# Thealexbarney/VGAudio

Hardware: AMD Instinct MI355X
Metric: Msamples/s encoded (GC-ADPCM, 4096 ch) at 1/2/4/8 GPUs; % HBM roofline (higher is better)
Workload: dtype int32; 1 GPU; BASELINE configs[1]: 4096 mono channels x 48 kHz x 60 s GC-ADPCM coefficient search + encode per GPU; parallelism=units sharded x1, channels_per_gpu=4096, samples_per_channel=2880000, bit_exact_channels_checked=0

## Files before the change

### vgaudio_amd/csrc/gc_encode_core.hpp

```cpp
#pragma once
#include <cstdint>

#if defined(__HIPCC__)
#define VGA_HD __host__ __device__ __forceinline__
#else
#define VGA_HD inline
#endif

#if defined(__HIP_DEVICE_COMPILE__)
#define VGA_MUL24(a, b) __mul24((a), (b))
#define VGA_OPAQUE(v) asm("" : "+v"(v))
#define VGA_OPAQUE_S(v) asm("" : "+s"(v))
static __device__ __forceinline__ uint32_t vga_square24(int e)
{
    uint32_t r;
    asm("v_mul_i32_i24 %0, %1, %1" : "=v"(r) : "v"(e));
    return r;
}
#else
#define VGA_MUL24(a, b) ((a) * (b))
#define VGA_OPAQUE(v) ((void)0)
#define VGA_OPAQUE_S(v) ((void)0)
#endif

// ... 173 lines not shown
    const float f = (float)d;
    if (f >= 2147483648.0f) return 2147483647;
    return (int)f;
#endif
}

VGA_HD uint32_t pack16(int lo, int hi) { return ((uint32_t)lo & 0xFFFFu) | ((uint32_t)hi << 16); }
VGA_HD int pair_lo(uint32_t v) { return (int)(int16_t)(v & 0xFFFFu); }
VGA_HD int pair_hi(uint32_t v) { return (int)v >> 16; }
VGA_HD int dot2_i16(uint32_t a, uint32_t b, int acc)
{
#if defined(__HIP_DEVICE_COMPILE__)
    typedef short s16x2 __attribute__((ext_vector_type(2)));
    return __builtin_amdgcn_sdot2(__builtin_bit_cast(s16x2, a), __builtin_bit_cast(s16x2, b), acc, true);
#else
    const int64_t v = (int64_t)pair_lo(a) * pair_lo(b) + (int64_t)pair_hi(a) * pair_hi(b) + (int64_t)acc;
    return v > 2147483647ll ? 2147483647 : (v < -2147483648ll ? (int)-2147483648ll : (int)v);
#endif
}
VGA_HD uint32_t sat_pack16(int lo, int hi)
{
#if defined(__HIP_DEVICE_COMPILE__)
    return __builtin_bit_cast(uint32_t, __builtin_amdgcn_cvt_pk_i16(lo, hi));
#else
    return pack16(clamp16i(lo), clamp16i(hi));
#endif
}
VGA_HD uint32_t pk_sub_sat_i16(uint32_t a, uint32_t b)
{
#if defined(__HIP_DEVICE_COMPILE__)
    typedef short s16x2 __attribute__((ext_vector_type(2)));
    return __builtin_bit_cast(uint32_t, __builtin_elementwise_sub_sat(__builtin_bit_cast(s16x2, a), __builtin_bit_cast(s16x2, b)));
#else
    return pack16(clamp16i(pair_lo(a) - pair_lo(b)), clamp16i(pair_hi(a) - pair_hi(b)));
#endif
}
VGA_HD int dot2_i16_wrap(uint32_t a, uint32_t b)
{
#if defined(__HIP_DEVICE_COMPILE__)
    typedef short s16x2 __attribute__((ext_vector_type(2)));
    return __builtin_amdgcn_sdot2(__builtin_bit_cast(s16x2, a), __builtin_bit_cast(s16x2, b), 0, false);
#else
    return (int)((uint32_t)(pair_lo(a) * pair_lo(b)) + (uint32_t)(pair_hi(a) * pair_hi(b)));
#endif
}
VGA_HD int numer_adjust(int N, int D_is_pos)
{
    VGA_OPAQUE(D_is_pos);
    return (int)((uint32_t)N + (uint32_t)VGA_MUL24(D_is_pos, 2047));
}
VGA_HD int head_distance_numer(int in2048p, int P)
{
    const int N = (int)((uint32_t)in2048p - (uint32_t)P);
    return numer_adjust(N, (int)((uint32_t)(1024 - P) >> 31)) >> 11;
}
VGA_HD void pack_row(const int (&x)[16], uint32_t (&xw)[7])
{
#if defined(__HIP_DEVICE_COMPILE__)
#pragma unroll
#endif
    for (int i = 0; i < 7; i++) xw[i] = pack16(x[2 + 2 * i], x[3 + 2 * i]);
}
VGA_HD void unpack_row(const uint32_t (&xw)[7], uint32_t hist, int (&x)[16])
{
    x[0] = pair_lo(hist);
    x[1] = pair_hi(hist);
#if defined(__HIP_DEVICE_COMPILE__)
#pragma unroll
#endif
    for (int i = 0; i < 7; i++) { x[2 + 2 * i] = pair_lo(xw[i]); x[3 + 2 * i] = pair_hi(xw[i]); }
}

VGA_HD int predicted_p1024(uint32_t h, uint32_t cpair)
{
    int k1024 = 1024;
    VGA_OPAQUE_S(k1024);
    return dot2_i16(h, cpair, k1024);
}
template <bool WIDE_TOTAL, bool NO_ROUND = false, bool HAVE_P0 = false>
VGA_HD PassOut pass_fast_core_t(const uint32_t (&xw)[7], uint32_t hist, const int (&in2048p)[14], int c0, int c1, int scale_power,
                                int P0 = 0)
{
    PassOut r;
    uint64_t total64 = 0;
    const int k = scale_power + 11;
    const int km11 = scale_power;
    int bias = (1 << (k - 1)) - 1;
    VGA_OPAQUE(bias);
    const uint32_t cpair = pack16(c1, c0);
    int k1024 = 1024;
    VGA_OPAQUE_S(k1024);
    int total = 0;
    int umax = 0, umin = 0;
    int u_prev = 0;
    uint32_t h = hist;
    int w_prev = pair_hi(hist);
#if defined(__HIP_DEVICE_COMPILE__)
#pragma unroll
#endif
    for (int s = 0; s < 14; s++) {
        const int P = (HAVE_P0 && s == 0) ? P0 : dot2_i16(h, cpair, k1024);
        const int d = (int)((uint32_t)in2048p[s] - (uint32_t)P);
        const int rd = NO_ROUND ? d : round_through_f32(d);
        const int u = (int)((uint32_t)rd + (uint32_t)bias + ((uint32_t)d >> 31)) >> k;
        const int q = imin(imax(u, -8), 7);
        if (s & 1) {
            umax = imax(imax(umax, u_prev), u);
            umin = imin(imin(umin, u_prev), u);
        }
        u_prev = u;
        r.q[s] = q;
        const int w = (P >> 11) + (int)((uint32_t)q << km11);
        h = sat_pack16(w_prev, w);
        w_prev = w;
        if (WIDE_TOTAL) {
            const int e = ((s & 1) ? pair_hi(xw[s >> 1]) : pair_lo(xw[s >> 1])) - pair_hi(h);
#if defined(__HIP_DEVICE_COMPILE__)
            total64 += (uint64_t)vga_square24(e);
#else
            total64 += (uint64_t)((int64_t)e * (int64_t)e);
#endif
        } else if (s & 1) {
            const uint32_t epk = pk_sub_sat_i16(xw[s >> 1], h);
            total = dot2_i16(epk, epk, total);
        }
    }
    r.hist_pair = h;
    const int ov = imax(imax(umax - 7, -8 - umin), 0);
    const int ac0 = c0 < 0 ? -c0 : c0, ac1 = c1 < 0 ? -c1 : c1;
    r.exact = ac0 + ac1 <= 32767 && (WIDE_TOTAL || (ov <= 12383 && (((2 * ov + 1) << (k - 11)) <= 24766)));
    r.total = WIDE_TOTAL ? total64 : (uint64_t)(uint32_t)total;
    r.max_overflow = ov;
    r.o12 = pair_lo(h); r.o13 = pair_hi(h);
    return r;
}
VGA_HD PassOut pass_fast_core(const uint32_t (&xw)[7], uint32_t hist, const int (&in2048p)[14], int c0, int c1, int scale_power)
{
    return pass_fast_core_t<false>(xw, hist, in2048p, c0, c1, scale_power);
}
VGA_HD PassOut pass_fast_core_no_round(const uint32_t (&xw)[7], uint32_t hist, const int (&in2048p)[14], int c0, int c1,
                                       int scale_power)
{
    return pass_fast_core_t<false, true>(xw, hist, in2048p, c0, c1, scale_power);
}
VGA_HD bool pass_no_round_is_exact(int scale_power, int max_overflow)
{
    return scale_power <= 9 && max_overflow < (1 << (13 - scale_power)) - 8;
}
VGA_HD PassOut pass_fast_core_wide(const uint32_t (&xw)[7], uint32_t hist, const int (&in2048p)[14], int c0, int c1,
                                   int scale_power)
{
    return pass_fast_core_t<true>(xw, hist, in2048p, c0, c1, scale_power);
}
constexpr uint64_t PACKED_SUM_CAP = 1ull << 28;
VGA_HD bool needs_exact_sum(uint64_t total, bool known_exact) { return !known_exact && total >= PACKED_SUM_CAP; }
VGA_HD PassOut pass_fast_core(const int (&x)[16], uint32_t hist, const int (&in2048p)[14], int c0, int c1, int scale_power)
{
    uint32_t xw[7];
    pack_row(x, xw);
    return pass_fast_core_t<false>(xw, hist, in2048p, c0, c1, scale_power);
}
VGA_HD PassOut pass_fast_core_no_round(const int (&x)[16], uint32_t hist, const int (&in2048p)[14], int c0, int c1,
                                       int scale_power)
{
    uint32_t xw[7];
    pack_row(x, xw);
    return pass_fast_core_t<false, true>(xw, hist, in2048p, c0, c1, scale_power);
}
VGA_HD PassOut pass_fast_core_wide(const int (&x)[16], uint32_t hist, const int (&in2048p)[14], int c0, int c1,
                                   int scale_power)
{
    uint32_t xw[7];
    pack_row(x, xw);
    return pass_fast_core_t<true>(xw, hist, in2048p, c0, c1, scale_power);
}
template <bool NO_ROUND>
VGA_HD PassOut pass_fast_core_exact_sum(const int (&x)[16], const int (&in2048p)[14], int c0, int c1, int scale_power)
{
    uint32_t xw[7];
    pack_row(x, xw);
    const uint32_t hist = pack16(x[0], x[1]);
    PassOut r = pass_fast_core_t<false, NO_ROUND>(xw, hist, in2048p, c0, c1, scale_power);
    const int ac0 = c0 < 0 ? -c0 : c0, ac1 = c1 < 0 ? -c1 : c1;
    if (ac0 + ac1 <= 32767 && needs_exact_sum(r.total, r.exact))
        r.total = pass_fast_core_t<true>(xw, hist, in2048p, c0, c1, scale_power).total;
    return r;
}
VGA_HD PassOut pass_fast_core(const int (&x)[16], const int (&)[14], const int (&in2048p)[14], int c0, int c1, int scale_power)
{
    return pass_fast_core_exact_sum<false>(x, in2048p, c0, c1, scale_power);
}
VGA_HD PassOut pass_fast_core_no_round(const int (&x)[16], const int (&)[14], const int (&in2048p)[14], int c0, int c1,
                                       int scale_power)
{
    return pass_fast_core_exact_sum<true>(x, in2048p, c0, c1, scale_power);
}
VGA_HD PassOut pass_fast_core_wide(const int (&x)[16], const int (&)[14], const int (&in2048p)[14], int c0, int c1,
                                   int scale_power)
{
    return pass_fast_core_wide(x, pack16(x[0], x[1]), in2048p, c0, c1, scale_power);
}

VGA_HD PassOut pass_fast(const int (&x)[16], int c0, int c1, int scale_power)
{
    int in2048p[14];
#if defined(__HIP_DEVICE_COMPILE__)
#pragma unroll
#endif
    for (int s = 0; s < 14; s++) in2048p[s] = x[s + 2] * 2048 + 1024;
    return pass_fast_core(x, pack16(x[0], x[1]), in2048p, c0, c1, scale_power);
}

struct Resolve {
    bool final_a;
    bool final_b;
    int resume_sp;
};

VGA_HD Resolve resolve_candidates(int s1, int ov_a, int ov_b)
{
    Resolve z;
    z.final_a = z.final_b = false;
    z.resume_sp = 0;
    const int sp_a = apply_bumps(s1, ov_a);
    if (!(sp_a < 12 && ov_a > 1)) { z.final_a = true; return z; }
    if (sp_a != s1) { z.resume_sp = sp_a; return z; }
    const int s2 = s1 + 1;
    const int sp_b = apply_bumps(s2, ov_b);
    if (!(sp_b < 12 && ov_b > 1)) { z.final_b = true; return z; }
    z.resume_sp = sp_b;
    return z;
}

VGA_HD Resolve resolve_candidates_nobump(int s1, int ov_a, int ov_b)
{
    Resolve z;
    z.final_a = !(s1 < 12 && ov_a > 1);
    z.final_b = !z.final_a && !(s1 + 1 < 12 && ov_b > 1);
    z.resume_sp = s1 + 1;
    return z;
}

VGA_HD PassOut resume_passes_core(const int (&x)[16], const int (&in2048p)[14], int c0, int c1, int scale_power,
                                  int &final_sp)
{
    PassOut r;
    bool at_max;
    do {
        scale_power++;
        at_max = scale_power >= 12;
        r = pass_fast_core(x, pack16(x[0], x[1]), in2048p, c0, c1, scale_power);
        if (!r.exact) r = pass_literal(x, c0, c1, scale_power);
        scale_power = apply_bumps(scale_power, r.max_overflow);
    } while (scale_power < 12 && r.max_overflow > 1 && !at_max);
    final_sp = scale_power;
    return r;
}

VGA_HD PassOut resume_passes(const int (&x)[16], int c0, int c1, int scale_power, int &final_sp)
{
    PassOut r;
    bool at_max;
    do {
        scale_power++;
        at_max = scale_power >= 12;
        r = pass_fast(x, c0, c1, scale_power);
        if (!r.exact) r = pass_literal(x, c0, c1, scale_power);
        scale_power = apply_bumps(scale_power, r.max_overflow);
    } while (scale_power < 12 && r.max_overflow > 1 && !at_max);
    final_sp = scale_power;
    return r;
}

}
}
```

### vgaudio_amd/csrc/gc_encode_kernel.hip

```cpp
#include "common.hpp"
#include "gc_encode_core.hpp"
#include "gcadpcm_kernels.hpp"
#include "seams.hpp"

#include <cstdio>
#include <cstdlib>

namespace vga {
namespace gc {

constexpr int DPP_QUAD_XOR1 = 0xB1;
constexpr int DPP_QUAD_XOR2 = 0x4E;
constexpr int DPP_ROW_HALF_MIRROR = 0x141;
constexpr int DPP_ROW_MIRROR = 0x140;

template <int CTRL>
__device__ __forceinline__ int dpp(int v)
{
    return __builtin_amdgcn_update_dpp(0, v, CTRL, 0xF, 0xF, true);
}

__device__ __forceinline__ unsigned umin32(unsigned a, unsigned b) { return a < b ? a : b; }

template <class Op>
__device__ __forceinline__ unsigned row16_reduce(unsigned v, Op op)
{
    v = op(v, (unsigned)dpp<DPP_QUAD_XOR1>((int)v));
    v = op(v, (unsigned)dpp<DPP_QUAD_XOR2>((int)v));
    v = op(v, (unsigned)dpp<DPP_ROW_HALF_MIRROR>((int)v));
    v = op(v, (unsigned)dpp<DPP_ROW_MIRROR>((int)v));
    return v;
}


#ifdef VGA_DEBUG_TIMESTAMPS
__device__ unsigned long long g_vga_enc_ts[1 << 16];
extern "C" int vga_debug_encode_timestamps(unsigned long long *out, int n)
{
    return (int)hipMemcpyFromSymbol(out, HIP_SYMBOL(g_vga_enc_ts), (size_t)n * sizeof(unsigned long long));
}
#endif
__device__ unsigned long long g_vga_gc_stats[8];
extern "C" int vga_testing_gc_encode_stats(unsigned long long *out8, int reset)
{
    if (hipDeviceSynchronize() != hipSuccess) return -1;
    if (out8 && hipMemcpyFromSymbol(out8, HIP_SYMBOL(g_vga_gc_stats), 8 * sizeof(unsigned long long)) != hipSuccess) return -1;
#ifdef VGA_GC_STATS
    if (out8) out8[7] = 1;
#else
    if (out8) out8[7] = 0;
#endif
    if (reset) {
        const unsigned long long zero[8] = {0, 0, 0, 0, 0, 0, 0, 0};
        if (hipMemcpyToSymbol(HIP_SYMBOL(g_vga_gc_stats), zero, sizeof zero) != hipSuccess) return -1;
    }
    return 0;
}
constexpr int SW = 2;
constexpr int ENC_THREADS = 64 * (SW + 1);
#ifndef VGA_GC_ENCODER_PRIO
#define VGA_GC_ENCODER_PRIO 3
#endif
#ifndef VGA_GC_HELPER_PRIO
#define VGA_GC_HELPER_PRIO 0
#endif
template <int CPW>
struct Lay {
    static constexpr int CS = CPW * SW;
    static constexpr int TF = 64 / CS;
};
template <int CS, int TF>
struct GcTileT {
    uint32_t xw[CS][TF][8];
    int in2048p[CS][TF][16];
    uint32_t pre[CS][TF][8];
};
typedef short short2v __attribute__((ext_vector_type(2)));
struct XW7 { uint32_t v[7]; };

#define VGA_COLD __device__ __forceinline__

VGA_COLD int prescan_sequential_cold(XW7 xs, uint32_t hist, int c0, int c1)
{
    int x[16];
    unpack_row(xs.v, hist, x);
    return prescan_sequential(x, c0, c1);
}

#ifdef VGA_GC_R05_COLD
#define VGA_COLD_OPAQUE(v) ((void)0)
#else
#define VGA_COLD_OPAQUE(v) VGA_OPAQUE(v)
#endif
struct ColdState {
    uint32_t xw[7];
    int mp[14];
    uint32_t hist;
    int c0, c1, s1;
    int generic, start, drop, wide, resume;
    int bump_a, ov_a, ov_b;
};
struct ColdOut { PassOut r; int final_sp; int fin; int sum_exact; };
__device__ __forceinline__
ColdOut encode_frame_cold(ColdState st, PassOut r, int final_sp, int fin)
{
    uint32_t xw[7];
    int mp[14];
#pragma unroll
    for (int i = 0; i < 7; i++) xw[i] = st.xw[i];
#pragma unroll
    for (int i = 0; i < 14; i++) mp[i] = st.mp[i];
    int sum_exact = 0;
    if (st.drop) fin = 0;
    if (__any(st.generic != 0)) {
        if (st.generic) {
            int xg[16];
            unpack_row(xw, st.hist, xg);
#pragma unroll
            for (int i = 0; i < 16; i++) VGA_COLD_OPAQUE(xg[i]);
            const int start = st.start != -100 ? st.start
                                               : (st.bump_a ? apply_bumps(st.s1, st.ov_a) : apply_bumps(st.s1 + 1, st.ov_b));
            r = resume_passes(xg, st.c0, st.c1, start, final_sp);
            fin = 1;
            sum_exact = 1;
        }
    }
    if (st.wide) fin = 1;
    if (__any(st.resume != 0)) {
        if (st.resume) {
            int sp = st.s1 + 1;
            for (;;) {
                sp++;
#if defined(VGA_GC_NO_FAST_PASSES) || defined(VGA_GC_NO_FAST_THIRD)
                bool short_pass = false;
#else
                bool short_pass = !__any(sp > 9);
#endif
                if (short_pass) {
                    r = pass_fast_core_no_round(xw, st.hist, mp, st.c0, st.c1, sp);
                    short_pass = !__any(!pass_no_round_is_exact(sp, r.max_overflow));
                }
                if (!short_pass) r = pass_fast_core(xw, st.hist, mp, st.c0, st.c1, sp);
                const bool cap = sp >= 12;
                if ((unsigned)r.max_overflow > (cap ? 3u : 248u)) {
                    int xg[16];
                    unpack_row(xw, st.hist, xg);
#pragma unroll
                    for (int i = 0; i < 16; i++) VGA_COLD_OPAQUE(xg[i]);
                    r = resume_passes(xg, st.c0, st.c1, sp - 1, final_sp);
                    sum_exact = 1;
                    break;
                }
                final_sp = sp;
                if (cap || r.max_overflow <= 1) break;
            }
            fin = 1;
        }
    }
    ColdOut o;
    o.r = r;
    o.final_sp = final_sp;
    o.fin = fin;
    o.sum_exact = sum_exact;
    return o;
}

template <bool REPAIR, int CPW, bool RAGGED>
__device__ __forceinline__ void gc_encode_piece(
    const int bx, const int by,
    const int16_t *__restrict__ pcm, int64_t pcm_pitch, int nch, int total_samples, const Pieces seg,
    const int16_t *__restrict__ coefs, const int16_t *__restrict__ hist1,
    const int16_t *__restrict__ hist2, uint8_t *__restrict__ adpcm, int64_t adpcm_pitch, int16_t *__restrict__ seg_state,
    const int *__restrict__ first_open, const Ragged &rg)
{
    constexpr bool repair = REPAIR;
    constexpr int CS = Lay<CPW>::CS, TF = Lay<CPW>::TF;
    using GcTile = GcTileT<CS, TF>;
    int64_t first_frame = seg.first(by);
    int repair_piece = 0;
    if (repair) {
        int k = SEAM_OPEN_LIMIT;
        for (int g = 0; g < CS; g++) {
            const int slot = bx * CS + g;
            if (slot < nch) {
                const int c = RAGGED ? rg.order[slot] : slot;
                k = first_open[c] < k ? first_open[c] : k;
            }
        }
        if (!is_open(k)) return;
        repair_piece = k;
        first_frame = seg.first(k);
    }
    const int total_wg = RAGGED ? rg.length[rg.order[bx * CS]] : total_samples;
    if (first_frame * 14 >= total_wg) return;
    const int64_t piece_samples = repair ? (int64_t)0x7fffffff : (int64_t)seg.frames(by) * 14;
    auto piece_samples_of = [&](int total) {
        const int64_t rem = (int64_t)total - first_frame * 14;
        return (int)(rem < 0 ? 0 : (rem < piece_samples ? rem : piece_samples));
    };
    pcm += first_frame * 14;
    adpcm += first_frame * 8;
    __shared__ GcTile s_tile[2];
    __shared__ int4 s_out[2][CS][TF][4];
    __shared__ int s_ncold[SW];
    const int tid = threadIdx.x;
    const int wave = tid >> 6;
    const bool helper = wave == SW;
    const int lane = tid & 63;
    constexpr int LPC = 64 / CPW;
    int grp = helper ? lane / TF : wave * CPW + lane / LPC;
    const int l16 = lane & (LPC - 1);
    const int hfr = lane % TF;
    const int slot_raw = bx * CS + grp;
    const bool live = slot_raw < nch;
    const int slot = live ? slot_raw : nch - 1;
    const int ch = RAGGED ? rg.order[slot] : slot;
    const int16_t *src = pcm + (RAGGED ? rg.pcm_off[ch] : (int64_t)ch * pcm_pitch);
    uint8_t *dst = adpcm + (RAGGED ? rg.adpcm_off[ch] : (int64_t)ch * adpcm_pitch);

    const int sample_count = piece_samples_of(RAGGED ? rg.length[ch] : total_samples);
    const int full_frames = sample_count / 14;
    const int tail = sample_count - full_frames * 14;
    const int frames = full_frames + (tail ? 1 : 0);
    const int frames_wg = RAGGED ? (piece_samples_of(total_wg) + 13) / 14 : frames;
    const int tiles = (frames_wg + TF - 1) / TF;

    if (helper) {
        __builtin_amdgcn_s_setprio(VGA_GC_HELPER_PRIO);
        uint32_t cpk[8];
#pragma unroll
        for (int p = 0; p < 8; p++)
            cpk[p] = (uint32_t)(uint16_t)coefs[ch * 16 + 2 * p + 1] | ((uint32_t)(uint16_t)coefs[ch * 16 + 2 * p] << 16);
        auto prepare = [&](int tile) {
            const int fr = RAGGED ? imax(imin(tile * TF + hfr, frames - 1), 0) : imin(tile * TF + hfr, frames - 1);
            int in[14];
            uint32_t w[7];
            if (fr < full_frames) {
                const uint32_t *p32 = reinterpret_cast<const uint32_t *>(src + (int64_t)fr * 14);
#pragma unroll
                for (int i = 0; i < 7; i++) w[i] = p32[i];
#pragma unroll
                for (int i = 0; i < 7; i++) {
                    in[2 * i] = (int)(int16_t)(w[i] & 0xFFFF);
                    in[2 * i + 1] = (int)w[i] >> 16;
                }
            } else {
#pragma unroll
                for (int s = 0; s < 14; s++) in[s] = (s < tail) ? (int)src[(int64_t)fr * 14 + s] : 0;
#pragma unroll
                for (int i = 0; i < 7; i++) w[i] = (uint32_t)(in[2 * i] & 0xFFFF) | ((uint32_t)in[2 * i + 1] << 16);
            }
            GcTile &T = s_tile[tile & 1];
            uint4 *xr = reinterpret_cast<uint4 *>(&T.xw[grp][hfr][0]);
            xr[0] = make_uint4(w[0], w[1], w[2], w[3]);
            xr[1] = make_uint4(w[4], w[5], w[6], 0u);
            int4 *qr = reinterpret_cast<int4 *>(&T.in2048p[grp][hfr][0]);
            qr[0] = make_int4(in[0] * 2048 + 1024, in[1] * 2048 + 1024, in[2] * 2048 + 1024, in[3] * 2048 + 1024);
            qr[1] = make_int4(in[4] * 2048 + 1024, in[5] * 2048 + 1024, in[6] * 2048 + 1024, in[7] * 2048 + 1024);
            qr[2] = make_int4(in[8] * 2048 + 1024, in[9] * 2048 + 1024, in[10] * 2048 + 1024, in[11] * 2048 + 1024);
            qr[3] = make_int4(in[12] * 2048 + 1024, in[13] * 2048 + 1024, 0, 0);
            uint32_t pair[12];
#pragma unroll
            for (int k = 0; k < 12; k++)
                pair[k] = (k & 1) ? __builtin_amdgcn_alignbit(w[(k + 1) / 2], w[(k - 1) / 2], 16) : w[k / 2];
            uint32_t pre[8];
#pragma unroll
            for (int p = 0; p < 8; p++) {
                int dmax = 0, dmin = 0;
#ifdef VGA_GC_ABLATE_HELPER_PRESCAN
                dmax = in[2 + p] & 1023;
                dmin = -(in[3 + p] & 1023);
#else
#pragma unroll
                for (int k = 0; k < 12; k++) {
                    const int predicted = div2048(__builtin_amdgcn_sdot2(__builtin_bit_cast(short2v, pair[k]),
                                                                         __builtin_bit_cast(short2v, cpk[p]), 0, false));
                    const int d = in[k + 2] - predicted;
                    dmax = imax(dmax, d);
                    dmin = imin(dmin, d);
                }
#endif
                pre[p] = (uint32_t)(clamp16i(dmax) & 0xFFFF) | ((uint32_t)clamp16i(dmin) << 16);
            }
            uint4 *pr = reinterpret_cast<uint4 *>(&T.pre[grp][hfr][0]);
            pr[0] = make_uint4(pre[0], pre[1], pre[2], pre[3]);
            pr[1] = make_uint4(pre[4], pre[5], pre[6], pre[7]);
        };
        auto flush = [&](int tile) {
            const int fr = tile * TF + hfr;
            if (!live || fr >= frames) return;
            const int4 *rec = &s_out[tile & 1][grp][hfr][0];
            const int4 r0 = rec[0], r1 = rec[1], r2 = rec[2], r3 = rec[3];
            const int q[14] = {r0.x, r0.y, r0.z, r0.w, r1.x, r1.y, r1.z, r1.w, r2.x, r2.y, r2.z, r2.w, r3.x, r3.y};
            uint2 v;
            pack_frame(q, r3.z, r3.w, v.x, v.y);
            if (fr < full_frames) {
                *reinterpret_cast<uint2 *>(dst + (int64_t)fr * 8) = v;
            } else {
                const int nbytes = (tail + 2 + 1) / 2;
                const uint64_t both = ((uint64_t)v.y << 32) | v.x;
                for (int b = 0; b < nbytes; b++) dst[(int64_t)fr * 8 + b] = (uint8_t)(both >> (8 * b));
            }
        };
        if (tiles > 0) prepare(0);
        __syncthreads();
        for (int tile = 0; tile < tiles; tile++) {
            if (tile + 1 < tiles) prepare(tile + 1);
            if (tile > 0) flush(tile - 1);
            __syncthreads();
        }
        if (tiles > 0) flush(tiles - 1);
        return;
    }

    __builtin_amdgcn_s_setprio(VGA_GC_ENCODER_PRIO);
    int p = CPW == 4 ? l16 >> 1 : l16;
    const bool cand_b = CPW == 4 && (l16 & 1) != 0;
    const int c0 = coefs[ch * 16 + 2 * p];
    const int c1 = coefs[ch * 16 + 2 * p + 1];
    const bool coef_ok = (c0 < 0 ? -c0 : c0) + (c1 < 0 ? -c1 : c1) <= 32767;
    int h0 = hist2 ? hist2[ch] : 0;
    int h1 = hist1 ? hist1[ch] : 0;
    if (repair) {
        h0 = seg_state[((int64_t)(repair_piece - 1) * nch + ch) * 2];
        h1 = seg_state[((int64_t)(repair_piece - 1) * nch + ch) * 2 + 1];
    } else if (by > 0 && (!RAGGED || frames > 0)) {
        h0 = src[-2];
        h1 = src[-1];
    }
    uint32_t hpk = pack16(h0, h1);

    if (lane == 0) s_ncold[wave] = 0;
    struct Row { uint32_t xw[7]; int mp[14]; uint32_t pre; };
    auto read_row = [&](const GcTile &T, int j, Row &R) {
        const uint4 *xr = reinterpret_cast<const uint4 *>(&T.xw[grp][j][0]);
        const uint4 a0 = xr[0], a1 = xr[1];
        asm volatile("" ::"v"(a1.w));
        uint32_t *xw = R.xw;
        xw[0] = a0.x; xw[1] = a0.y; xw[2] = a0.z; xw[3] = a0.w; xw[4] = a1.x; xw[5] = a1.y; xw[6] = a1.z;
        const int4 *qr = reinterpret_cast<const int4 *>(&T.in2048p[grp][j][0]);
        const int4 e0 = qr[0], e1 = qr[1], e2 = qr[2], e3 = qr[3];
        asm volatile("" ::"v"(e3.z), "v"(e3.w));
        int *mp = R.mp;
        mp[0] = e0.x; mp[1] = e0.y; mp[2] = e0.z; mp[3] = e0.w; mp[4] = e1.x; mp[5] = e1.y; mp[6] = e1.z; mp[7] = e1.w;
        mp[8] = e2.x; mp[9] = e2.y; mp[10] = e2.z; mp[11] = e2.w; mp[12] = e3.x; mp[13] = e3.y;
        R.pre = T.pre[grp][j][p];
    };
    auto pack = [](const uint32_t (&xw)[7]) {
        XW7 xs;
#pragma unroll
        for (int i = 0; i < 7; i++) xs.v[i] = xw[i];
        return xs;
    };
    const uint32_t cpk = pack16(c1, c0);
    const bool head_numer = __builtin_amdgcn_ballot_w64(!coef_ok) == 0;
    auto prescan_head = [&](const Row &R, int &d0, int &d1, int &P0) __attribute__((always_inline)) {
        P0 = predicted_p1024(hpk, cpk);
        if (__builtin_expect(head_numer, 1)) {
            d0 = head_distance_numer(R.mp[0], P0);
            d1 = head_distance_numer(R.mp[1], predicted_p1024(__builtin_amdgcn_alignbit(R.xw[0], hpk, 16), cpk));
        } else {
            d0 = pair_lo(R.xw[0]) - div2048(dot2_i16_wrap(hpk, cpk));
            d1 = pair_hi(R.xw[0]) - div2048(dot2_i16_wrap(__builtin_amdgcn_alignbit(R.xw[0], hpk, 16), cpk));
        }
    };
    auto first_scale = [&](const Row &R, int d0, int d1) __attribute__((always_inline)) -> int {
        const int dmax = imax(imax((int)(int16_t)(R.pre & 0xFFFF), d0), d1);
        const int dmin = imin(imin((int)R.pre >> 16, d0), d1);
        int sum, pos;
        int s1 = first_scale_power_nt(dmax, dmin, sum, pos);
        if (__builtin_expect(__builtin_amdgcn_ballot_w64(sum == 0) != 0, 0)) {
            if (sum == 0 && first_scale_tie(pos)) s1 = first_scale_power_from_md(prescan_sequential_cold(pack(R.xw), hpk, c0, c1));
        }
        return s1;
    };

    auto encode_frame = [&](Row &R, int buf, int j, bool upd) {
        const uint32_t (&xw)[7] = R.xw;
        int s1, P0;
        {
            int d0, d1;
            prescan_head(R, d0, d1, P0);
            s1 = first_scale(R, d0, d1);
        }
        int final_sp = imin(s1 + (cand_b ? 1 : 0), 12);
        const bool at_cap = final_sp >= 12;
        const unsigned ov_limit = at_cap ? 3u : 248u;
        PassOut r = pass_fast_core_t<false, false, true>(xw, hpk, R.mp, c0, c1, final_sp, P0);
        const bool rare = !coef_ok || (!at_cap && (unsigned)r.max_overflow > ov_limit);
        const int eff = at_cap ? 0 : r.max_overflow;
        const int eff_other = dpp<DPP_QUAD_XOR1>(eff);
        bool fin = eff < 2 && (eff_other | (cand_b ? 0 : 2)) >= 2;
        const bool resume = !cand_b && imin(eff, eff_other) >= 2;
        const bool inexact = fin && at_cap && (unsigned)r.max_overflow > ov_limit;
        constexpr unsigned SAT = (1u << 28) - 1;
        auto argmin32 = [&](const PassOut &r, bool fin, bool &sat) __attribute__((always_inline)) -> int {
            const unsigned tot = umin32((unsigned)(r.total >> 32) ? SAT : (unsigned)r.total, SAT);
            const unsigned key = fin ? ((tot << 4) | (unsigned)l16) : 0xFFFFFFFFu;
            const unsigned best = row16_reduce(key, [](unsigned a, unsigned b) { return a < b ? a : b; });
            sat = __any((best >> 4) >= SAT);
            return (int)(best & 15u);
        };
        auto argmin64 = [&](uint64_t total, bool fin) __attribute__((always_inline)) -> int {
            uint64_t key = fin ? ((total << 4) | (uint64_t)l16) : ~0ull;
#define VGA_MIN64_STAGE(CTRL)                                                          \
            {                                                                          \
                const unsigned olo = (unsigned)dpp<CTRL>((int)(uint32_t)key);          \
                const unsigned ohi = (unsigned)dpp<CTRL>((int)(uint32_t)(key >> 32));  \
                const uint64_t okey = ((uint64_t)ohi << 32) | olo;                     \
                key = okey < key ? okey : key;                                         \
            }
            VGA_MIN64_STAGE(DPP_QUAD_XOR1)
            VGA_MIN64_STAGE(DPP_QUAD_XOR2)
            VGA_MIN64_STAGE(DPP_ROW_HALF_MIRROR)
            VGA_MIN64_STAGE(DPP_ROW_MIRROR)
#undef VGA_MIN64_STAGE
            return (int)(key & 15u);
        };
        auto commit = [&](const PassOut &r, int final_sp, int winner) __attribute__((always_inline)) {
            const bool won = l16 == winner;
            const unsigned pay = row16_reduce(won ? r.hist_pair : 0u,
                                              [](unsigned a, unsigned b) { return a | b; });
            if (won) {
                int4 *rec = &s_out[buf][grp][j][0];
                rec[0] = make_int4(r.q[0], r.q[1], r.q[2], r.q[3]);
                rec[1] = make_int4(r.q[4], r.q[5], r.q[6], r.q[7]);
                rec[2] = make_int4(r.q[8], r.q[9], r.q[10], r.q[11]);
                rec[3] = make_int4(r.q[12], r.q[13], p, final_sp);
            }
            if (!RAGGED || upd) hpk = pay;
        };
        bool sat = false;
        const int winner32 = argmin32(r, fin && !inexact, sat);
        if (__builtin_expect(__any(rare || resume || inexact) || sat, 0)) {
#ifdef VGA_GC_STATS
            if (lane == 0) atomicAdd(&s_ncold[wave], 1);
#endif
            ColdState st;
#pragma unroll
            for (int i = 0; i < 7; i++) st.xw[i] = xw[i];
#pragma unroll
            for (int i = 0; i < 14; i++) st.mp[i] = R.mp[i];
            st.hist = hpk;
            st.c0 = c0; st.c1 = c1; st.s1 = s1;
            const bool redo = __any(rare);
            st.generic = redo && !cand_b; st.start = s1 - 1; st.drop = redo && cand_b;
            st.wide = !redo && inexact; st.resume = !redo && resume;
            st.bump_a = 0; st.ov_a = 0; st.ov_b = 0;
            const ColdOut o = encode_frame_cold(st, r, final_sp, fin);
            bool sat2 = false;
            int winner = argmin32(o.r, o.fin != 0, sat2);
            if (sat2) {
                uint64_t total = o.r.total;
                if (o.fin != 0 && needs_exact_sum(total, o.sum_exact != 0))
                    total = pass_fast_core_wide(xw, hpk, R.mp, c0, c1, o.final_sp).total;
                winner = argmin64(total, o.fin != 0);
            }
            commit(o.r, o.final_sp, winner);
        } else
            commit(r, final_sp, winner32);
    };

    auto encode_frame8 = [&](Row &R, int buf, int j, bool upd) {
        const uint32_t (&xw)[7] = R.xw;
        int s1, P0;
        {
            int d0, d1;
            prescan_head(R, d0, d1, P0);
            s1 = first_scale(R, d0, d1);
        }
        const int sp_a = imin(s1, 12), sp_b = imin(s1 + 1, 12);
        PassOut ra, rb;
#ifdef VGA_GC_NO_FAST_PASSES
        bool short_passes = false;
#else
        bool short_passes = !__any(sp_b > 9);
#endif
        if (short_passes) {
            rb = pass_fast_core_t<false, true, true>(xw, hpk, R.mp, c0, c1, sp_b, P0);
            ra = pass_fast_core_t<false, true, true>(xw, hpk, R.mp, c0, c1, sp_a, P0);
            const bool trusted = !coef_ok || (pass_no_round_is_exact(sp_a, ra.max_overflow) && pass_no_round_is_exact(sp_b, rb.max_overflow));
            short_passes = !__any(!trusted);
        }
        if (!short_passes) {
            rb = pass_fast_core_t<false, false, true>(xw, hpk, R.mp, c0, c1, sp_b, P0);
            ra = pass_fast_core_t<false, false, true>(xw, hpk, R.mp, c0, c1, sp_a, P0);
        }
        const bool cap_a = sp_a >= 12, cap_b = sp_b >= 12;
        const int eff_a = cap_a ? 0 : ra.max_overflow, eff_b = cap_b ? 0 : rb.max_overflow;
        const bool fin_a = eff_a < 2;
        const bool bump_a = !cap_a && (unsigned)ra.max_overflow > 248u;
        const bool bump_b = !fin_a && !cap_b && (unsigned)rb.max_overflow > 248u;
        const bool generic = !coef_ok || bump_a || bump_b;
        const bool inexact = !generic && (fin_a ? (cap_a && (unsigned)ra.max_overflow > 3u) : (cap_b && (unsigned)rb.max_overflow > 3u));
#ifdef VGA_GC_ABLATE_THIRD_TRIPS
        const bool resume = false;
#else
        const bool resume = !generic && !fin_a && eff_b >= 2;
#endif
        PassOut r;
#pragma unroll
        for (int i = 0; i < 14; i++) r.q[i] = fin_a ? ra.q[i] : rb.q[i];
        r.total = fin_a ? ra.total : rb.total;
        r.hist_pair = fin_a ? ra.hist_pair : rb.hist_pair;
        r.max_overflow = fin_a ? ra.max_overflow : rb.max_overflow;
        r.o12 = r.o13 = 0;
        r.exact = true;
        const int final_sp = fin_a ? sp_a : sp_b;
        constexpr unsigned SAT = (1u << 28) - 1;
        auto argmin32 = [&](const PassOut &r, bool fin, bool &sat) __attribute__((always_inline)) -> int {
            const unsigned tot = umin32((unsigned)(r.total >> 32) ? SAT : (unsigned)r.total, SAT);
            unsigned key = fin ? ((tot << 3) | (unsigned)p) : 0xFFFFFFFFu;
            key = umin32(key, (unsigned)dpp<DPP_QUAD_XOR1>((int)key));
            key = umin32(key, (unsigned)dpp<DPP_QUAD_XOR2>((int)key));
            key = umin32(key, (unsigned)dpp<DPP_ROW_HALF_MIRROR>((int)key));
            sat = __any((key >> 3) >= SAT);
            return (int)(key & 7u);
        };
        auto argmin64 = [&](uint64_t total, bool fin) __attribute__((always_inline)) -> int {
            uint64_t key = fin ? ((total << 3) | (uint64_t)p) : ~0ull;
#define VGA_MIN64_STAGE(CTRL)                                                          \
            {                                                                          \
                const unsigned olo = (unsigned)dpp<CTRL>((int)(uint32_t)key);          \
                const unsigned ohi = (unsigned)dpp<CTRL>((int)(uint32_t)(key >> 32));  \
                const uint64_t okey = ((uint64_t)ohi << 32) | olo;                     \
                key = okey < key ? okey : key;                                         \
            }
            VGA_MIN64_STAGE(DPP_QUAD_XOR1)
            VGA_MIN64_STAGE(DPP_QUAD_XOR2)
            VGA_MIN64_STAGE(DPP_ROW_HALF_MIRROR)
#undef VGA_MIN64_STAGE
            return (int)(key & 7u);
        };
        auto commit = [&](const PassOut &r, int final_sp, int winner) __attribute__((always_inline)) {
            const bool won = p == winner;
            unsigned pay = won ? r.hist_pair : 0u;
            pay |= (unsigned)dpp<DPP_QUAD_XOR1>((int)pay);
            pay |= (unsigned)dpp<DPP_QUAD_XOR2>((int)pay);
            pay |= (unsigned)dpp<DPP_ROW_HALF_MIRROR>((int)pay);
            if (won) {
                int4 *rec = &s_out[buf][grp][j][0];
                rec[0] = make_int4(r.q[0], r.q[1], r.q[2], r.q[3]);
                rec[1] = make_int4(r.q[4], r.q[5], r.q[6], r.q[7]);
                rec[2] = make_int4(r.q[8], r.q[9], r.q[10], r.q[11]);
                rec[3] = make_int4(r.q[12], r.q[13], p, final_sp);
            }
            if (!RAGGED || upd) hpk = pay;
        };
        bool sat = false;
        const int winner32 = argmin32(r, !(generic || resume || inexact), sat);
        if (__builtin_expect(__any(generic || resume || inexact) || sat, 0)) {
#ifdef VGA_GC_STATS
            if (lane == 0) atomicAdd(&s_ncold[wave], 1);
#endif
            ColdState st;
#pragma unroll
            for (int i = 0; i < 7; i++) st.xw[i] = xw[i];
#pragma unroll
            for (int i = 0; i < 14; i++) st.mp[i] = R.mp[i];
            st.hist = hpk;
            st.c0 = c0; st.c1 = c1; st.s1 = s1;
            st.generic = generic; st.drop = 0; st.wide = inexact; st.resume = resume;
#ifdef VGA_GC_R05_COLD
            st.start = !coef_ok ? s1 - 1 : (bump_a ? apply_bumps(s1, ra.max_overflow) : apply_bumps(s1 + 1, rb.max_overflow));
#else
            st.start = !coef_ok ? s1 - 1 : -100;
#endif
            st.bump_a = bump_a; st.ov_a = ra.max_overflow; st.ov_b = rb.max_overflow;
            const ColdOut o = encode_frame_cold(st, r, final_sp, (generic || resume) ? 0 : 1);
            bool sat2 = false;
            int winner = argmin32(o.r, o.fin != 0, sat2);
            if (sat2) {
                uint64_t total = o.r.total;
                if (o.fin != 0 && needs_exact_sum(total, o.sum_exact != 0))
                    total = pass_fast_core_wide(xw, hpk, R.mp, c0, c1, o.final_sp).total;
                winner = argmin64(total, o.fin != 0);
            }
            commit(o.r, o.final_sp, winner);
        } else
            commit(r, final_sp, winner32);
    };
    auto encode_one = [&](Row &R, int buf, int j, bool upd) __attribute__((always_inline)) {
        if constexpr (CPW == 4) encode_frame(R, buf, j, upd);
        else encode_frame8(R, buf, j, upd);
    };

#ifdef VGA_DEBUG_TIMESTAMPS
    if (!repair && tid == 0 && gridDim.y != 1) g_vga_enc_ts[2 * ((blockIdx.y * gridDim.x + blockIdx.x) & 32767)] = wall_clock64();
#endif
    __syncthreads();
    for (int tile = 0; tile < tiles; tile++) {
        const int buf = tile & 1;
        const int nf = imin(TF, frames_wg - tile * TF);
        const int left = frames - tile * TF;
#ifndef VGA_GC_NO_TILE_REDERIVE
        {
            int l = lane;
            asm volatile("" : "+v"(l));
            grp = wave * CPW + l / LPC;
            p = CPW == 4 ? (l & (LPC - 1)) >> 1 : (l & (LPC - 1));
        }
#endif
        const GcTile &T = s_tile[buf];
        Row RA, RB;
        read_row(T, 0, RA);
#pragma unroll 1
        for (int j = 0; j < nf; j += 2) {
            read_row(T, imin(j + 1, TF - 1), RB);
            encode_one(RA, buf, j, j < left);
            if (j + 1 < nf) {
                read_row(T, imin(j + 2, TF - 1), RA);
                encode_one(RB, buf, j + 1, j + 1 < left);
            }
        }
        __syncthreads();
    }
    if (seg_state && !repair && live && l16 == 0) {
        int16_t *st = seg_state + ((int64_t)by * nch + ch) * 2;
        st[0] = (int16_t)pair_lo(hpk);
        st[1] = (int16_t)pair_hi(hpk);
    }
    if (lane == 0) {
        atomicAdd(&g_vga_gc_stats[3], (unsigned long long)frames_wg);
        atomicAdd(&g_vga_gc_stats[4], (unsigned long long)s_ncold[wave]);
        if (wave == 0) atomicAdd(&g_vga_gc_stats[6], 1ull);
    }
#ifdef VGA_DEBUG_TIMESTAMPS
    if (!repair && tid == 0 && gridDim.y != 1) g_vga_enc_ts[2 * ((blockIdx.y * gridDim.x + blockIdx.x) & 32767) + 1] = wall_clock64();
#endif
}


template <bool REPAIR, int CPW, bool RAGGED>
__global__ __launch_bounds__(ENC_THREADS) __attribute__((amdgpu_waves_per_eu(3, 3))) void gc_encode_kernel(
    const int16_t *__restrict__ pcm, int64_t pcm_pitch, int nch, int total_samples, const Pieces seg,
    const int16_t *__restrict__ coefs, const int16_t *__restrict__ hist1,
    const int16_t *__restrict__ hist2, uint8_t *__restrict__ adpcm, int64_t adpcm_pitch, int16_t *__restrict__ seg_state,
    const int *__restrict__ first_open, const Ragged rg)
{
    gc_encode_piece<REPAIR, CPW, RAGGED>(blockIdx.x, blockIdx.y, pcm, pcm_pitch, nch, total_samples, seg, coefs, hist1, hist2, adpcm,
                                         adpcm_pitch, seg_state, first_open, rg);
}

__device__ __forceinline__ void store_frame_bytes(uint8_t *dst, uint32_t d0, uint32_t d1, int nbytes)
{
    const uint64_t bits = ((uint64_t)d1 << 32) | d0;
    for (int b = 0; b < nbytes; b++) dst[b] = (uint8_t)(bits >> (8 * b));
}

template <int LPC>
__device__ __forceinline__ void seam_run(const int16_t *__restrict__ src, uint8_t *__restrict__ dst, int c0, int c1, bool coef_ok,
                                         int pr, int ch, int k, int64_t f0, int total_samples, int piece_frames, int max_frames, int force_open,
                                         int &h0, int &h1, int g2, int g1, bool &open, int &frames_run)
{
    static_assert(LPC == 8 || LPC == 16, "a lane per predictor, or per (predictor, candidate)");
    const bool cand_b = LPC == 16 && (threadIdx.x & 1) != 0;
    const int full_frames = total_samples / 14;
    const int64_t f_end = imin((int)imin((int)(f0 + piece_frames), (int)(f0 + max_frames)), full_frames);
    const int64_t f_last = full_frames > 0 ? full_frames - 1 : 0;
    auto fetch = [&](int64_t f, uint32_t (&w)[7], uint2 &old) {
        const int64_t fc = f < f_last ? f : f_last;
        const uint32_t *p32 = reinterpret_cast<const uint32_t *>(src + fc * 14);
#pragma unroll
        for (int i = 0; i < 7; i++) w[i] = p32[i];
        old = *reinterpret_cast<const uint2 *>(dst + fc * 8);
    };
    uint32_t w[7], wn[7];
    uint2 old, oldn;
    fetch(f0, w, old);
    for (int64_t f = f0; ; f++) {
        const bool in_range = f < f_end;
        if (!__any(open && in_range)) break;
        const bool act = open && in_range;
        frames_run += act ? 1 : 0;
        fetch(f + 1, wn, oldn);
        int x[16], mp[14];
        x[0] = h0;
        x[1] = h1;
        const uint32_t hpk = pack16(h0, h1);
#pragma unroll
        for (int i = 0; i < 7; i++) {
            x[2 + 2 * i] = (int)(int16_t)(w[i] & 0xFFFF);
            x[3 + 2 * i] = (int)w[i] >> 16;
        }
#pragma unroll
        for (int i = 0; i < 14; i++) mp[i] = x[2 + i] * 2048 + 1024;
        {
            const int ps = (int)(old.x & 0xFFu);
            const int scale = (1 << (ps & 0xF)) * 2048;
            const int pred = (ps >> 4) & 7;
            const int k1 = __shfl(c0, LPC == 16 ? 2 * pred : pred, LPC), k2 = __shfl(c1, LPC == 16 ? 2 * pred : pred, LPC);
            const uint64_t bits = ((uint64_t)old.y << 32) | old.x;
#pragma unroll
            for (int s2 = 0; s2 < 14; s2++) {
                const int byte = (int)((bits >> (8 * (1 + (s2 >> 1)))) & 0xFFu);
                const int nib = (s2 & 1) ? (byte & 0xF) : (byte >> 4);
                const int v = clamp16i((k1 * g1 + k2 * g2 + scale * ((nib ^ 8) - 8) + 1024) >> 11);
                g2 = g1;
                g1 = v;
            }
        }
        int s1;
        {
            int dmax = 0, dmin = 0;
            prescan_range(x, c0, c1, 0, 14, dmax, dmin);
            s1 = first_scale_power_from_range(dmax, dmin);
            if (s1 == -100) s1 = first_scale_power_from_md(prescan_sequential(x, c0, c1));
        }
        const int sp_a = imin(s1, 12), sp_b = imin(s1 + 1, 12);
        PassOut r;
        int final_sp;
        bool fin = true;
        if (LPC == 8) {
        const PassOut rb = pass_fast_core(w, hpk, mp, c0, c1, sp_b);
        const PassOut ra = pass_fast_core(w, hpk, mp, c0, c1, sp_a);
        const bool cap_a = sp_a >= 12, cap_b = sp_b >= 12;
        const bool rare = !coef_ok || (unsigned)ra.max_overflow > (cap_a ? 2u : 248u) || (unsigned)rb.max_overflow > (cap_b ? 2u : 248u);
        const int eff_a = cap_a ? 0 : ra.max_overflow, eff_b = cap_b ? 0 : rb.max_overflow;
        const bool fin_a = eff_a < 2;
        const bool resume = !fin_a && eff_b >= 2;
#pragma unroll
        for (int i = 0; i < 14; i++) r.q[i] = fin_a ? ra.q[i] : rb.q[i];
        r.total = fin_a ? ra.total : rb.total;
        r.hist_pair = fin_a ? ra.hist_pair : rb.hist_pair;
        final_sp = fin_a ? sp_a : sp_b;
        if (__any(rare || resume)) {
            if (rare || resume) {
                const PassOut rc = resume_passes(x, c0, c1, rare ? s1 - 1 : s1 + 1, final_sp);
// ... 506 lines not shown
```

Baseline: 75060 Msamples/s.

## Rewrite GC-ADPCM scale pass with biased offset arithmetic, med3 clamp and deferred error sum

Adds a new pass core that stores input rows with a large constant offset, so the rounding difference can be computed with a borrow-based unsigned subtract and the quantised nibble clamped with a single med3 instruction. The two candidate short passes no longer compute error sums. They record the reconstructed sample pairs instead, and the squared-error sum is computed once for the selected pass. Packing now masks nibbles modulo 16, and the coefficient-validity threshold is tightened to fit the offset scheme. This is meant to cut per-sample ALU work and avoid a redundant error reduction in the hot loop. The cost is carrying seven extra registers per pass and tighter exactness bounds.

```diff
diff --git a/vgaudio_amd/csrc/gc_encode_core.hpp b/vgaudio_amd/csrc/gc_encode_core.hpp
--- a/vgaudio_amd/csrc/gc_encode_core.hpp
+++ b/vgaudio_amd/csrc/gc_encode_core.hpp
@@ -349,6 +349,138 @@
 {
     return pass_fast_core_t<true>(xw, hist, in2048p, c0, c1, scale_power);
 }
+constexpr int PASS_B_OFF = 1 << 30;
+constexpr int PASS_B_COEF_SUM_MAX = 30720;
+struct PassOutB {
+    int q2[14];
+    uint64_t total;
+    int max_overflow;
+    unsigned hist_pair;
+    bool exact;
+    uint32_t pairs[7];
+};
+VGA_HD bool pass_b_coef_ok(int c0, int c1)
+{
+    return (c0 < 0 ? -c0 : c0) + (c1 < 0 ? -c1 : c1) <= PASS_B_COEF_SUM_MAX;
+}
+VGA_HD int pass_b_z(int scale_power) { return 1 << (19 - scale_power); }
+VGA_HD int pass_b_row(int in) { return in * 2048 + 1024 + PASS_B_OFF; }
+VGA_HD int predicted_b(uint32_t h, uint32_t cpair)
+{
+    int kacc = 1024 + PASS_B_OFF;
+    VGA_OPAQUE_S(kacc);
+    return dot2_i16(h, cpair, kacc);
+}
+VGA_HD int head_distance_numer_b(int in_b, int P_b)
+{
+    const int N = (int)((uint32_t)in_b - (uint32_t)P_b);
+    return numer_adjust(N, (int)((uint32_t)(1024 + PASS_B_OFF - P_b) >> 31)) >> 11;
+}
+VGA_HD int med3_i32(int v, int lo, int hi)
+{
+#if defined(__HIP_DEVICE_COMPILE__)
+    int r;
+    asm("v_med3_i32 %0, %1, %2, %3" : "=v"(r) : "v"(v), "v"(lo), "v"(hi));
+    return r;
+#else
+    return imin(imax(v, lo), hi);
+#endif
+}
+VGA_HD uint32_t sub_borrow_u32(uint32_t a, uint32_t b, uint32_t &borrow)
+{
+    uint32_t d;
+    borrow = __builtin_usub_overflow(a, b, &d) ? 1u : 0u;
+    return d;
+}
+VGA_HD uint32_t error_sum_pairs(const uint32_t (&xw)[7], const uint32_t (&pairs)[7])
+{
+    int total = 0;
+#if defined(__HIP_DEVICE_COMPILE__)
+#pragma unroll
+#endif
+    for (int i = 0; i < 7; i++) {
+        const uint32_t epk = pk_sub_sat_i16(xw[i], pairs[i]);
+        total = dot2_i16(epk, epk, total);
+    }
+    return (uint32_t)total;
+}
+template <bool NO_ROUND, bool HAVE_P0 = false, bool WITH_SUM = true>
+VGA_HD PassOutB pass_fast_core_b(const uint32_t (&xw)[7], uint32_t hist, const int (&in_b)[14], int c0, int c1, int scale_power,
+                                 int P0_b = 0)
+{
+    PassOutB r;
+    const int k = scale_power + 11;
+    const int km11 = scale_power;
+    int bias2 = (1 << (k - 1)) - 1 - PASS_B_OFF;
+    VGA_OPAQUE(bias2);
+    const int nz = -(1 << 19) >> scale_power;
+    const int q_lo = nz - 8, q_hi = nz + 7;
+    const uint32_t cpair = pack16(c1, c0);
+    int kacc = 1024 + PASS_B_OFF;
+    VGA_OPAQUE_S(kacc);
+    int total = 0;
+    int umax = nz, umin = nz;
+    int u_prev = nz;
+    uint32_t h = hist;
+    int w_prev = pair_hi(hist);
+#if defined(__HIP_DEVICE_COMPILE__)
+#pragma unroll
+#endif
+    for (int s = 0; s < 14; s++) {
+        const int P = (HAVE_P0 && s == 0) ? P0_b : dot2_i16(h, cpair, kacc);
+        uint32_t b;
+        const int d = (int)sub_borrow_u32((uint32_t)in_b[s], (uint32_t)P, b);
+        const int rd = NO_ROUND ? d : round_through_f32(d);
+        const int u2 = (int)((uint32_t)rd + (uint32_t)bias2 + b) >> k;
+        const int q2 = med3_i32(u2, q_lo, q_hi);
+        if (s & 1) {
+            umax = imax(imax(umax, u_prev), u2);
+            umin = imin(imin(umin, u_prev), u2);
+        }
+        u_prev = u2;
+        r.q2[s] = q2;
+        const int w = (P >> 11) + (int)((uint32_t)q2 << km11);
+        h = sat_pack16(w_prev, w);
+        w_prev = w;
+        if (s & 1) {
+            if (WITH_SUM) {
+                const uint32_t epk = pk_sub_sat_i16(xw[s >> 1], h);
+                total = dot2_i16(epk, epk, total);
+            } else
+                r.pairs[s >> 1] = h;
+        }
+    }
+    r.hist_pair = h;
+    const int ov = imax(imax(umax - q_hi, q_lo - umin), 0);
+    r.exact = pass_b_coef_ok(c0, c1) && ov <= 12383 && (((2 * ov + 1) << (k - 11)) <= 24766);
+    r.total = (uint64_t)(uint32_t)total;
+    r.max_overflow = ov;
+    return r;
+}
+VGA_HD void pack_frame_mod16(const int (&q)[14], int predictor, int scale_power, uint32_t &d0, uint32_t &d1)
+{
+    uint32_t wa = 0, wb = 0;
+#if defined(__HIP_DEVICE_COMPILE__)
+#pragma unroll
+#endif
+    for (int s = 0; s < 14; s++) {
+        if (s < 6) wa = (wa << 4) | ((uint32_t)q[s] & 15u);
+        else       wb = (wb << 4) | ((uint32_t)q[s] & 15u);
+    }
+    const uint32_t header = (uint32_t)((predictor << 4) | (scale_power & 0xF));
+    d0 = bswap32((header << 24) | wa);
+    d1 = bswap32(wb);
+}
+VGA_HD PassOutB as_pass_b(const PassOut &r)
+{
+    PassOutB o;
+#if defined(__HIP_DEVICE_COMPILE__)
+#pragma unroll
+#endif
+    for (int s = 0; s < 14; s++) o.q2[s] = r.q[s];
+    o.total = r.total; o.max_overflow = r.max_overflow; o.hist_pair = r.hist_pair; o.exact = r.exact;
+    return o;
+}
 constexpr uint64_t PACKED_SUM_CAP = 1ull << 28;
 VGA_HD bool needs_exact_sum(uint64_t total, bool known_exact) { return !known_exact && total >= PACKED_SUM_CAP; }
 VGA_HD PassOut pass_fast_core(const int (&x)[16], uint32_t hist, const int (&in2048p)[14], int c0, int c1, int scale_power)
diff --git a/vgaudio_amd/csrc/gc_encode_kernel.hip b/vgaudio_amd/csrc/gc_encode_kernel.hip
--- a/vgaudio_amd/csrc/gc_encode_kernel.hip
+++ b/vgaudio_amd/csrc/gc_encode_kernel.hip
@@ -100,9 +100,9 @@
     int generic, start, drop, wide, resume;
     int bump_a, ov_a, ov_b;
 };
-struct ColdOut { PassOut r; int final_sp; int fin; int sum_exact; };
+struct ColdOut { PassOutB r; int final_sp; int fin; int sum_exact; };
 __device__ __forceinline__
-ColdOut encode_frame_cold(ColdState st, PassOut r, int final_sp, int fin)
+ColdOut encode_frame_cold(ColdState st, PassOutB r, int final_sp, int fin)
 {
     uint32_t xw[7];
     int mp[14];
@@ -120,7 +120,7 @@
             for (int i = 0; i < 16; i++) VGA_COLD_OPAQUE(xg[i]);
             const int start = st.start != -100 ? st.start
                                                : (st.bump_a ? apply_bumps(st.s1, st.ov_a) : apply_bumps(st.s1 + 1, st.ov_b));
-            r = resume_passes(xg, st.c0, st.c1, start, final_sp);
+            r = as_pass_b(resume_passes(xg, st.c0, st.c1, start, final_sp));
             fin = 1;
             sum_exact = 1;
         }
@@ -137,17 +137,17 @@
                 bool short_pass = !__any(sp > 9);
 #endif
                 if (short_pass) {
-                    r = pass_fast_core_no_round(xw, st.hist, mp, st.c0, st.c1, sp);
+                    r = pass_fast_core_b<true>(xw, st.hist, mp, st.c0, st.c1, sp);
                     short_pass = !__any(!pass_no_round_is_exact(sp, r.max_overflow));
                 }
-                if (!short_pass) r = pass_fast_core(xw, st.hist, mp, st.c0, st.c1, sp);
+                if (!short_pass) r = pass_fast_core_b<false>(xw, st.hist, mp, st.c0, st.c1, sp);
                 const bool cap = sp >= 12;
                 if ((unsigned)r.max_overflow > (cap ? 3u : 248u)) {
                     int xg[16];
                     unpack_row(xw, st.hist, xg);
 #pragma unroll
                     for (int i = 0; i < 16; i++) VGA_COLD_OPAQUE(xg[i]);
-                    r = resume_passes(xg, st.c0, st.c1, sp - 1, final_sp);
+                    r = as_pass_b(resume_passes(xg, st.c0, st.c1, sp - 1, final_sp));
                     sum_exact = 1;
                     break;
                 }
@@ -255,10 +255,10 @@
             xr[0] = make_uint4(w[0], w[1], w[2], w[3]);
             xr[1] = make_uint4(w[4], w[5], w[6], 0u);
             int4 *qr = reinterpret_cast<int4 *>(&T.in2048p[grp][hfr][0]);
-            qr[0] = make_int4(in[0] * 2048 + 1024, in[1] * 2048 + 1024, in[2] * 2048 + 1024, in[3] * 2048 + 1024);
-            qr[1] = make_int4(in[4] * 2048 + 1024, in[5] * 2048 + 1024, in[6] * 2048 + 1024, in[7] * 2048 + 1024);
-            qr[2] = make_int4(in[8] * 2048 + 1024, in[9] * 2048 + 1024, in[10] * 2048 + 1024, in[11] * 2048 + 1024);
-            qr[3] = make_int4(in[12] * 2048 + 1024, in[13] * 2048 + 1024, 0, 0);
+            qr[0] = make_int4(pass_b_row(in[0]), pass_b_row(in[1]), pass_b_row(in[2]), pass_b_row(in[3]));
+            qr[1] = make_int4(pass_b_row(in[4]), pass_b_row(in[5]), pass_b_row(in[6]), pass_b_row(in[7]));
+            qr[2] = make_int4(pass_b_row(in[8]), pass_b_row(in[9]), pass_b_row(in[10]), pass_b_row(in[11]));
+            qr[3] = make_int4(pass_b_row(in[12]), pass_b_row(in[13]), 0, 0);
             uint32_t pair[12];
 #pragma unroll
             for (int k = 0; k < 12; k++)
@@ -293,7 +293,7 @@
             const int4 r0 = rec[0], r1 = rec[1], r2 = rec[2], r3 = rec[3];
             const int q[14] = {r0.x, r0.y, r0.z, r0.w, r1.x, r1.y, r1.z, r1.w, r2.x, r2.y, r2.z, r2.w, r3.x, r3.y};
             uint2 v;
-            pack_frame(q, r3.z, r3.w, v.x, v.y);
+            pack_frame_mod16(q, r3.z, r3.w, v.x, v.y);
             if (fr < full_frames) {
                 *reinterpret_cast<uint2 *>(dst + (int64_t)fr * 8) = v;
             } else {
@@ -318,7 +318,7 @@
     const bool cand_b = CPW == 4 && (l16 & 1) != 0;
     const int c0 = coefs[ch * 16 + 2 * p];
     const int c1 = coefs[ch * 16 + 2 * p + 1];
-    const bool coef_ok = (c0 < 0 ? -c0 : c0) + (c1 < 0 ? -c1 : c1) <= 32767;
+    const bool coef_ok = pass_b_coef_ok(c0, c1);
     int h0 = hist2 ? hist2[ch] : 0;
     int h1 = hist1 ? hist1[ch] : 0;
     if (repair) {
@@ -353,12 +353,18 @@
         return xs;
     };
     const uint32_t cpk = pack16(c1, c0);
+    auto wide_total = [&](const uint32_t (&xw)[7], const int (&mp)[14], int sp) -> uint64_t {
+        int row[14];
+#pragma unroll
+        for (int i = 0; i < 14; i++) row[i] = mp[i] - PASS_B_OFF;
+        return pass_fast_core_wide(xw, hpk, row, c0, c1, sp).total;
+    };
     const bool head_numer = __builtin_amdgcn_ballot_w64(!coef_ok) == 0;
     auto prescan_head = [&](const Row &R, int &d0, int &d1, int &P0) __attribute__((always_inline)) {
-        P0 = predicted_p1024(hpk, cpk);
+        P0 = predicted_b(hpk, cpk);
         if (__builtin_expect(head_numer, 1)) {
-            d0 = head_distance_numer(R.mp[0], P0);
-            d1 = head_distance_numer(R.mp[1], predicted_p1024(__builtin_amdgcn_alignbit(R.xw[0], hpk, 16), cpk));
+            d0 = head_distance_numer_b(R.mp[0], P0);
+            d1 = head_distance_numer_b(R.mp[1], predicted_b(__builtin_amdgcn_alignbit(R.xw[0], hpk, 16), cpk));
         } else {
             d0 = pair_lo(R.xw[0]) - div2048(dot2_i16_wrap(hpk, cpk));
             d1 = pair_hi(R.xw[0]) - div2048(dot2_i16_wrap(__builtin_amdgcn_alignbit(R.xw[0], hpk, 16), cpk));
@@ -386,7 +392,7 @@
         int final_sp = imin(s1 + (cand_b ? 1 : 0), 12);
         const bool at_cap = final_sp >= 12;
         const unsigned ov_limit = at_cap ? 3u : 248u;
-        PassOut r = pass_fast_core_t<false, false, true>(xw, hpk, R.mp, c0, c1, final_sp, P0);
+        PassOutB r = pass_fast_core_b<false, true>(xw, hpk, R.mp, c0, c1, final_sp, P0);
         const bool rare = !coef_ok || (!at_cap && (unsigned)r.max_overflow > ov_limit);
         const int eff = at_cap ? 0 : r.max_overflow;
         const int eff_other = dpp<DPP_QUAD_XOR1>(eff);
@@ -394,7 +400,7 @@
         const bool resume = !cand_b && imin(eff, eff_other) >= 2;
         const bool inexact = fin && at_cap && (unsigned)r.max_overflow > ov_limit;
         constexpr unsigned SAT = (1u << 28) - 1;
-        auto argmin32 = [&](const PassOut &r, bool fin, bool &sat) __attribute__((always_inline)) -> int {
+        auto argmin32 = [&](const PassOutB &r, bool fin, bool &sat) __attribute__((always_inline)) -> int {
             const unsigned tot = umin32((unsigned)(r.total >> 32) ? SAT : (unsigned)r.total, SAT);
             const unsigned key = fin ? ((tot << 4) | (unsigned)l16) : 0xFFFFFFFFu;
             const unsigned best = row16_reduce(key, [](unsigned a, unsigned b) { return a < b ? a : b; });
@@ -417,16 +423,16 @@
 #undef VGA_MIN64_STAGE
             return (int)(key & 15u);
         };
-        auto commit = [&](const PassOut &r, int final_sp, int winner) __attribute__((always_inline)) {
+        auto commit = [&](const PassOutB &r, int final_sp, int winner) __attribute__((always_inline)) {
             const bool won = l16 == winner;
             const unsigned pay = row16_reduce(won ? r.hist_pair : 0u,
                                               [](unsigned a, unsigned b) { return a | b; });
             if (won) {
                 int4 *rec = &s_out[buf][grp][j][0];
-                rec[0] = make_int4(r.q[0], r.q[1], r.q[2], r.q[3]);
-                rec[1] = make_int4(r.q[4], r.q[5], r.q[6], r.q[7]);
-                rec[2] = make_int4(r.q[8], r.q[9], r.q[10], r.q[11]);
-                rec[3] = make_int4(r.q[12], r.q[13], p, final_sp);
+                rec[0] = make_int4(r.q2[0], r.q2[1], r.q2[2], r.q2[3]);
+                rec[1] = make_int4(r.q2[4], r.q2[5], r.q2[6], r.q2[7]);
+                rec[2] = make_int4(r.q2[8], r.q2[9], r.q2[10], r.q2[11]);
+                rec[3] = make_int4(r.q2[12], r.q2[13], p, final_sp);
             }
             if (!RAGGED || upd) hpk = pay;
         };
@@ -453,7 +459,7 @@
             if (sat2) {
                 uint64_t total = o.r.total;
                 if (o.fin != 0 && needs_exact_sum(total, o.sum_exact != 0))
-                    total = pass_fast_core_wide(xw, hpk, R.mp, c0, c1, o.final_sp).total;
+                    total = wide_total(xw, R.mp, o.final_sp);
                 winner = argmin64(total, o.fin != 0);
             }
             commit(o.r, o.final_sp, winner);
@@ -470,21 +476,21 @@
             s1 = first_scale(R, d0, d1);
         }
         const int sp_a = imin(s1, 12), sp_b = imin(s1 + 1, 12);
-        PassOut ra, rb;
+        PassOutB ra, rb;
 #ifdef VGA_GC_NO_FAST_PASSES
         bool short_passes = false;
 #else
         bool short_passes = !__any(sp_b > 9);
 #endif
         if (short_passes) {
-            rb = pass_fast_core_t<false, true, true>(xw, hpk, R.mp, c0, c1, sp_b, P0);
-            ra = pass_fast_core_t<false, true, true>(xw, hpk, R.mp, c0, c1, sp_a, P0);
+            rb = pass_fast_core_b<true, true, false>(xw, hpk, R.mp, c0, c1, sp_b, P0);
+            ra = pass_fast_core_b<true, true, false>(xw, hpk, R.mp, c0, c1, sp_a, P0);
             const bool trusted = !coef_ok || (pass_no_round_is_exact(sp_a, ra.max_overflow) && pass_no_round_is_exact(sp_b, rb.max_overflow));
             short_passes = !__any(!trusted);
         }
         if (!short_passes) {
-            rb = pass_fast_core_t<false, false, true>(xw, hpk, R.mp, c0, c1, sp_b, P0);
-            ra = pass_fast_core_t<false, false, true>(xw, hpk, R.mp, c0, c1, sp_a, P0);
+            rb = pass_fast_core_b<false, true, false>(xw, hpk, R.mp, c0, c1, sp_b, P0);
+            ra = pass_fast_core_b<false, true, false>(xw, hpk, R.mp, c0, c1, sp_a, P0);
         }
         const bool cap_a = sp_a >= 12, cap_b = sp_b >= 12;
         const int eff_a = cap_a ? 0 : ra.max_overflow, eff_b = cap_b ? 0 : rb.max_overflow;
@@ -498,17 +504,19 @@
 #else
         const bool resume = !generic && !fin_a && eff_b >= 2;
 #endif
-        PassOut r;
-#pragma unroll
-        for (int i = 0; i < 14; i++) r.q[i] = fin_a ? ra.q[i] : rb.q[i];
-        r.total = fin_a ? ra.total : rb.total;
-        r.hist_pair = fin_a ? ra.hist_pair : rb.hist_pair;
+        PassOutB r;
+#pragma unroll
+        for (int i = 0; i < 14; i++) r.q2[i] = fin_a ? ra.q2[i] : rb.q2[i];
+        uint32_t sel[7];
+#pragma unroll
+        for (int i = 0; i < 7; i++) sel[i] = fin_a ? ra.pairs[i] : rb.pairs[i];
+        r.total = error_sum_pairs(xw, sel);
+        r.hist_pair = sel[6];
         r.max_overflow = fin_a ? ra.max_overflow : rb.max_overflow;
-        r.o12 = r.o13 = 0;
         r.exact = true;
         const int final_sp = fin_a ? sp_a : sp_b;
         constexpr unsigned SAT = (1u << 28) - 1;
-        auto argmin32 = [&](const PassOut &r, bool fin, bool &sat) __attribute__((always_inline)) -> int {
+        auto argmin32 = [&](const PassOutB &r, bool fin, bool &sat) __attribute__((always_inline)) -> int {
             const unsigned tot = umin32((unsigned)(r.total >> 32) ? SAT : (unsigned)r.total, SAT);
             unsigned key = fin ? ((tot << 3) | (unsigned)p) : 0xFFFFFFFFu;
             key = umin32(key, (unsigned)dpp<DPP_QUAD_XOR1>((int)key));
@@ -532,7 +540,7 @@
 #undef VGA_MIN64_STAGE
             return (int)(key & 7u);
         };
-        auto commit = [&](const PassOut &r, int final_sp, int winner) __attribute__((always_inline)) {
+        auto commit = [&](const PassOutB &r, int final_sp, int winner) __attribute__((always_inline)) {
             const bool won = p == winner;
             unsigned pay = won ? r.hist_pair : 0u;
             pay |= (unsigned)dpp<DPP_QUAD_XOR1>((int)pay);
@@ -540,10 +548,10 @@
             pay |= (unsigned)dpp<DPP_ROW_HALF_MIRROR>((int)pay);
             if (won) {
                 int4 *rec = &s_out[buf][grp][j][0];
-                rec[0] = make_int4(r.q[0], r.q[1], r.q[2], r.q[3]);
-                rec[1] = make_int4(r.q[4], r.q[5], r.q[6], r.q[7]);
-                rec[2] = make_int4(r.q[8], r.q[9], r.q[10], r.q[11]);
-                rec[3] = make_int4(r.q[12], r.q[13], p, final_sp);
+                rec[0] = make_int4(r.q2[0], r.q2[1], r.q2[2], r.q2[3]);
+                rec[1] = make_int4(r.q2[4], r.q2[5], r.q2[6], r.q2[7]);
+                rec[2] = make_int4(r.q2[8], r.q2[9], r.q2[10], r.q2[11]);
+                rec[3] = make_int4(r.q2[12], r.q2[13], p, final_sp);
             }
             if (!RAGGED || upd) hpk = pay;
         };
@@ -573,7 +581,7 @@
             if (sat2) {
                 uint64_t total = o.r.total;
                 if (o.fin != 0 && needs_exact_sum(total, o.sum_exact != 0))
-                    total = pass_fast_core_wide(xw, hpk, R.mp, c0, c1, o.final_sp).total;
+                    total = wide_total(xw, R.mp, o.final_sp);
                 winner = argmin64(total, o.fin != 0);
             }
             commit(o.r, o.final_sp, winner);
```

New measurement: 78490 Msamples/s (median of 6 runs). +4.6%, better.
